# ShuhongChen/panic3d-anime-reconstruction

Hardware: AMD Instinct MI355X
Metric: rendered rays/sec at 512^2 img x 96 samples/ray (higher is better)
Workload: dtype f32

## Files before the change

### panic3d-anime-reconstruction_amd/csrc/p3d_importance.hpp

```cpp
#pragma once

#if defined(__HIPCC__)
#define P3D_IMP_FN __host__ __device__ __forceinline__
#define P3D_IMP_UNROLL _Pragma("unroll")
#else
#define P3D_IMP_FN inline
#define P3D_IMP_UNROLL
#endif

struct P3dFloatKey {
    P3D_IMP_FN static float mn(float a, float b) { return __builtin_fminf(a, b); }
    P3D_IMP_FN static float mx(float a, float b) { return __builtin_fmaxf(a, b); }
    P3D_IMP_FN static float neg(float a) { return -a; }
};

P3D_IMP_FN constexpr int p3d_pow2_ceil(int n) { int p = 1; while (p < n) p <<= 1; return p; }

template <int NR, typename K = P3dFloatKey, typename T>
P3D_IMP_FN void p3d_sort_merge_pass(T (&a)[NR], int pp) {
    constexpr int N = p3d_pow2_ceil(NR);
P3D_IMP_UNROLL
    for (int k = pp; k >= 1; k >>= 1) {
P3D_IMP_UNROLL
        for (int jj = k % pp; jj + k < N; jj += 2 * k) {
P3D_IMP_UNROLL
            for (int i = 0; i < k; ++i) {
                if (i + jj + k < NR && (i + jj) / (2 * pp) == (i + jj + k) / (2 * pp)) {
                    T x = a[i + jj], y = a[i + jj + k];
                    a[i + jj] = K::mn(x, y);
                    a[i + jj + k] = K::mx(x, y);
                }
            }
        }
    }
}
template <int NR, typename K = P3dFloatKey, typename T>
P3D_IMP_FN void p3d_sort_network(T (&a)[NR]) {
P3D_IMP_UNROLL
    for (int pp = 1; pp < p3d_pow2_ceil(NR); pp <<= 1) p3d_sort_merge_pass<NR, K>(a, pp);
}

template <typename K = P3dFloatKey, typename T>
P3D_IMP_FN void p3d_cross_half_exchange(T lo, T hi_neg, T& lo_out_neg, T& hi_out) {
    lo_out_neg = K::mx(K::neg(lo), hi_neg);
    hi_out = K::mx(lo, K::neg(hi_neg));
}

template <int H, typename K = P3dFloatKey, typename T>
P3D_IMP_FN void p3d_valley_merge(T (&a)[H]) {
    constexpr int N = p3d_pow2_ceil(H);
P3D_IMP_UNROLL
    for (int k = N / 2; k >= 1; k >>= 1) {
P3D_IMP_UNROLL
        for (int i = 0; i < H; ++i) {
            if ((i & k) == 0 && i + k < H) {
                T x = a[i], y = a[i + k];
                a[i] = K::mn(x, y);
                a[i + k] = K::mx(x, y);
            }
        }
    }
}

P3D_IMP_FN constexpr int p3d_half_rank(int H, int h, int i) { return h ? H + i : H - 1 - i; }

P3D_IMP_FN int p3d_merge_split_steps(int Sc, int Sf) {
    int n = Sc < Sf ? Sc : Sf, s = 0;
    while (n > 0) { ++s; n >>= 1; }
    return s;
}
template <typename RD>
P3D_IMP_FN int p3d_merge_split(RD rd, int Sc, int Sf, int D, int steps) {
    int lo = D - Sf > 0 ? D - Sf : 0, hi = D < Sc ? D : Sc;
    for (int s = 0; s < steps; ++s) {
        const int mid = (lo + hi) >> 1;
        const int cm = mid < Sc - 1 ? mid : Sc - 1, fm = D - mid - 1 < 0 ? 0 : (D - mid - 1 < Sf ? D - mid - 1 : Sf - 1);
        const bool behind = rd(false, fm) < rd(true, cm);
        const bool open = lo < hi;
        hi = (open && behind) ? mid : hi;
        lo = (open && !behind) ? mid + 1 : lo;
    }
    return lo;
}

template <typename RD, typename KN, typename PUT>
P3D_IMP_FN void p3d_merge_bits_half(RD rd, KN known, PUT put, int Sc, int Sf, int h) {
    const int S = Sc + Sf, D = S >> 1, qb = h ? D : 0, qe = h ? S : D;
    int ci = p3d_merge_split(rd, Sc, Sf, qb, p3d_merge_split_steps(Sc, Sf)), fi = qb - ci;
    const float inf = __builtin_inff();
    float ta = rd(true, ci < Sc ? ci : Sc - 1), tb = Sf > 0 ? rd(false, fi < Sf ? fi : Sf - 1) : inf;
    unsigned kw = 0u, sw = 0u;
    for (int it = 0; it < S - D; ++it) {
        const int q = qb + it;
        const bool mine = q < qe;
        const bool take_c = (ci < Sc) && (fi >= Sf || ta <= tb);
        const bool kn = known(take_c, take_c ? ci : fi, take_c ? ta : tb);
        kw |= (mine && kn) ? (1u << (q & 31)) : 0u;
        sw |= (mine && take_c) ? (1u << (q & 31)) : 0u;
        ci += take_c ? 1 : 0;
        fi += take_c ? 0 : 1;
        const int cq = ci < Sc ? ci : Sc - 1, fq = fi < Sf ? fi : (Sf > 0 ? Sf - 1 : 0);
        const float nv = rd(take_c, take_c ? cq : fq);
        ta = take_c ? nv : ta;
        tb = take_c ? tb : nv;
        if (mine && ((q & 31) == 31 || q == qe - 1)) {
            put(q >> 5, kw, sw);
            kw = 0u; sw = 0u;
        }
    }
}

#if defined(__HIPCC__)
template <int H>
__device__ __forceinline__ void p3d_sort_halves(float (&tf)[H], int h) {
    typedef uint32_t u32x2 __attribute__((ext_vector_type(2)));
    const uint32_t neg1 = h ? 0x80000000u : 0u;
P3D_IMP_UNROLL
    for (int i = 0; i < H; ++i) tf[i] = __builtin_bit_cast(float, __builtin_bit_cast(uint32_t, tf[i]) ^ neg1);
    p3d_sort_network<H>(tf);
P3D_IMP_UNROLL
    for (int i = 0; i < H; i += 2) {
        u32x2 in = __builtin_amdgcn_permlane32_swap(__builtin_bit_cast(uint32_t, tf[i]), __builtin_bit_cast(uint32_t, tf[i + 1]), false, false);
        const uint32_t in0 = in.x, in1 = in.y;
        float mn_neg, mx;
        p3d_cross_half_exchange(__builtin_bit_cast(float, in0), __builtin_bit_cast(float, in1), mn_neg, mx);
        u32x2 out = __builtin_amdgcn_permlane32_swap(__builtin_bit_cast(uint32_t, mn_neg), __builtin_bit_cast(uint32_t, mx), false, false);
        const uint32_t out0 = out.x, out1 = out.y;
        tf[i] = __builtin_bit_cast(float, out0);
        tf[i + 1] = __builtin_bit_cast(float, out1);
    }
    p3d_valley_merge<H>(tf);
}

template <typename RAW>
__device__ __forceinline__ float p3d_coarse_rank(RAW raw, int i, int Sc, bool wave_unsorted, bool wave_bad) {
    float a = raw(i);
    if (wave_unsorted) {
        if (!wave_bad) {
            const float lo = i > 0 ? raw(i - 1) : -__builtin_inff(), hi = i < Sc - 1 ? raw(i + 1) : __builtin_inff();
            a = lo > a ? lo : (a > hi ? hi : a);
        } else {
            for (int c = 0; c < Sc; ++c) {
                const float tv = raw(c);
                int r = 0;
                for (int x = 0; x < Sc; ++x) {
                    const float tx = raw(x);
                    r += (tx < tv || (tx == tv && x < c)) ? 1 : 0;
                }
                a = (r == i) ? tv : a;
            }
        }
    }
    return a;
}

template <typename TCS, typename FINE, typename KN, typename PUT>
__device__ __forceinline__ void p3d_merge_bits_ranks(TCS tc_sorted, FINE fine, KN known, PUT put, uint32_t fw0, uint32_t fw1, uint32_t fw2,
                                                     int Sc, int Sf, int h) {
    const int S = Sc + Sf, nmw = (S + 31) >> 5;
    uint32_t slw[6], knw[6];
P3D_IMP_UNROLL
    for (int w = 0; w < 6; ++w) { slw[w] = 0u; knw[w] = 0u; }
    const int Sch = ((Sc + 15) >> 4) << 3, ib = h * Sch;
    for (int i0 = 0; i0 < Sch; i0 += 8) {
        float tv[8];
        int pos[8];
P3D_IMP_UNROLL
        for (int q = 0; q < 8; ++q) { tv[q] = tc_sorted(ib + i0 + q < Sc ? ib + i0 + q : Sc - 1); pos[q] = 0; }
P3D_IMP_UNROLL
        for (int step = 64; step >= 1; step >>= 1) {
            float c[8];
P3D_IMP_UNROLL
            for (int q = 0; q < 8; ++q) c[q] = fine((pos[q] + step <= Sf) ? pos[q] + step - 1 : 0);
P3D_IMP_UNROLL
            for (int q = 0; q < 8; ++q) pos[q] = ((pos[q] + step <= Sf) && (c[q] < tv[q])) ? pos[q] + step : pos[q];
        }
P3D_IMP_UNROLL
        for (int q = 0; q < 8; ++q) {
            const int i = ib + i0 + q;
            const bool kn = known(i, tv[q]);
            const int P = i + pos[q], pw = (i < Sc) ? (P >> 5) : -1;
            const uint32_t b = 1u << (P & 31);
P3D_IMP_UNROLL
            for (int w = 0; w < 6; ++w) {
                slw[w] |= (pw == w) ? b : 0u;
                knw[w] |= (pw == w && kn) ? b : 0u;
            }
        }
    }
P3D_IMP_UNROLL
    for (int w = 0; w < 6; ++w) { slw[w] |= __shfl_xor(slw[w], 32); knw[w] |= __shfl_xor(knw[w], 32); }
    if (__builtin_amdgcn_ballot_w64((fw0 | fw1 | fw2) != 0u) != 0) {
        int fk = 0;
P3D_IMP_UNROLL
        for (int w = 0; w < 6; ++w) {
            if (w * 32 < S) {
                uint32_t kk = 0u;
                for (int b = 0; b < 32; ++b) {
                    const bool isf = !((slw[w] >> b) & 1u) && (w * 32 + b < S);
                    const uint32_t fwv = (fk < 32) ? fw0 : (fk < 64 ? fw1 : fw2);
                    kk |= (isf && ((fwv >> (fk & 31)) & 1u)) ? (1u << b) : 0u;
                    fk += isf ? 1 : 0;
                }
                knw[w] |= kk;
            }
        }
    }
P3D_IMP_UNROLL
    for (int w = 0; w < 6; ++w)
        if (w < nmw) put(w, knw[w], slw[w]);
}
#endif
```

### panic3d-anime-reconstruction_amd/csrc/p3d_kernels.hip

```cpp
#include <hip/hip_runtime.h>
#include <stddef.h>
#include <stdlib.h>
#include <string.h>

#include <atomic>
#include <type_traits>

#include "p3d_ray_phases.hpp"
#include "p3d_render_plan.hpp"
#include "p3d_phase_timing.hpp"

#define P3D_WAVES_PER_WG 4
#define P3D_WG (64 * P3D_WAVES_PER_WG)

__global__ __launch_bounds__(256) void k_planes_to_nhwc(const float* __restrict__ src, float* __restrict__ dst, int HW) {
    __shared__ float tile[32][65];
    const int p0 = blockIdx.x * 64;
    const size_t img = (size_t)blockIdx.y * 32 * HW;
    {
        int px = threadIdx.x & 63, c0 = threadIdx.x >> 6;
#pragma unroll
        for (int k = 0; k < 8; ++k) {
            int c = c0 + 4 * k;
            tile[c][px] = (p0 + px < HW) ? src[img + (size_t)c * HW + p0 + px] : 0.0f;
        }
    }
    __syncthreads();
    {
        int c = threadIdx.x & 31, q0 = threadIdx.x >> 5;
#pragma unroll
        for (int k = 0; k < 8; ++k) {
            int px = q0 + 8 * k;
            if (p0 + px < HW) dst[img + (size_t)(p0 + px) * 32 + c] = tile[c][px];
        }
    }
}

struct DecodeParams {
    const float* planes;
    const float* coords;
    const float *w0, *b0, *w1, *b1;
    float* out_sigma;
    float* out_rgb;
    unsigned char* out_cropmask;
    float mask_limit;
    long long M;
    long long tiles_per_img;
    long long ntiles;
    int H, W;
    int grid_n;
    long long grid_lo;
    float vsize, goff0, goff1, goff2;
    P3dDecodeCfg cfg;
};

P3D_DEV float p3d_fmod_pos(float a, float b) {
    const float q = __builtin_truncf(a / b);
    const float r = __builtin_fmaf(-q, b, a);
    return r < 0.0f ? r + b : r;
}

template <bool WANT_RGB, bool STAGED, bool FASTD>
__global__ __launch_bounds__(P3D_WG, 2) void k_decode_points(DecodeParams p) {
    static_assert(!(FASTD && WANT_RGB), "the tolerance-mode point decoder is density-only");
    extern __shared__ __attribute__((aligned(16))) float lds_alloc[];
    float* lds = FASTD ? lds_alloc - P3D_LDS_B0P : lds_alloc;
    p3d_load_mlp_to_lds(lds, p.w0, p.b0, p.w1, p.b1, !FASTD, !FASTD);
    if constexpr (FASTD) p3d_load_mlp_f16_to_lds(lds, p.w0, p.w1, false);
    __syncthreads();
    const int lane = threadIdx.x & 63, wave = threadIdx.x >> 6, j = lane & 31, h = lane >> 5;
    float* box = lds + (FASTD ? P3D_LDS_FAST_FLOATS : P3D_LDS_MLP_FLOATS) + 4 + (STAGED ? wave * P3D_BOX_FLOATS_PER_WAVE : 0);
    (void)box;
    P3dPlaneGeom g;
    g.halfW = 0.5f * (float)p.W; g.halfH = 0.5f * (float)p.H; g.fW = (float)p.W; g.fH = (float)p.H; g.W = p.W;
    g.plane_bytes = (uint32_t)p.H * (uint32_t)p.W * 128u;
    const long long stride = (long long)gridDim.x * P3D_WAVES_PER_WG;

    struct Tile {
        long long n, m;
        bool active, skip, any;
        float px, py, pz;
    };
    auto setup = [&](long long tile, Tile& t) {
        long long n = 0, tl = tile;
        if (p.tiles_per_img != p.ntiles) { n = tile / p.tiles_per_img; tl = tile - n * p.tiles_per_img; }
        t.n = n;
        t.m = tl * 32 + j;
        t.active = t.m < p.M;
        const long long mc = t.active ? t.m : p.M - 1;
        t.skip = false;
        if (p.coords) {
            const float* c = p.coords + ((size_t)n * p.M + mc) * 3;
            t.px = c[0]; t.py = c[1]; t.pz = c[2];
        } else {
            const unsigned idx = (unsigned)(p.grid_lo + mc);
            const float fn = (float)p.grid_n, f = (float)idx;
            const float s2 = (float)(idx % (unsigned)p.grid_n);
            const float q1 = f / fn;
            const float s1 = p3d_fmod_pos(q1, fn);
            const float s0 = p3d_fmod_pos(q1 / fn, fn);
            t.px = s0 * p.vsize + p.goff0; t.py = s1 * p.vsize + p.goff1; t.pz = s2 * p.vsize + p.goff2;
            if (p.out_cropmask) {
                const bool cropped = __builtin_fabsf(t.px) > p.mask_limit || __builtin_fabsf(t.pz) > p.mask_limit;
                if (t.active && h == 0) p.out_cropmask[t.m] = cropped ? 1 : 0;
                if (p.cfg.flags & P3D_FLAG_SKIP_CROPPED) t.skip = cropped;
            }
        }
        t.any = __builtin_amdgcn_ballot_w64(t.active && !t.skip) != 0;
    };
    auto resource = [&](long long n) {
        const unsigned nlo = __builtin_amdgcn_readfirstlane((unsigned)n);
        const float* base = p.planes + ((p.cfg.flags & P3D_FLAG_SHARED_PLANES) ? (size_t)0 : (size_t)nlo * 3 * (g.plane_bytes / 4));
        return __builtin_amdgcn_make_buffer_rsrc((void*)base, 0, 3 * g.plane_bytes, 0x00020000);
    };
    auto finish = [&](const Tile& t, float sigma, const f32x16& rgb) {
        if (t.skip) sigma = -1000.0f;
        if (t.active) {
            const size_t o = (size_t)t.n * p.M + t.m;
            if (h == 0) p.out_sigma[o] = sigma;
            if (WANT_RGB) {
                float* dst = p.out_rgb + o * 32 + 4 * h;
#pragma unroll
                for (int q = 0; q < 4; ++q)
                    *(f32x4*)(dst + 8 * q) = (f32x4){rgb[4 * q], rgb[4 * q + 1], rgb[4 * q + 2], rgb[4 * q + 3]};
            }
        }
    };

    long long tile = (long long)blockIdx.x * P3D_WAVES_PER_WG + wave;
    if constexpr (!STAGED) {
        for (; tile < p.ntiles; tile += stride) {
            Tile t;
            setup(tile, t);
            float sigma = -1000.0f;
            f32x16 rgb;
            if (t.any) {
                if constexpr (FASTD) p3d_decode_wave_fast<WANT_RGB, true>(lds, resource(t.n), g, p.cfg, t.px, t.py, t.pz, sigma, rgb, !t.skip);
                else p3d_decode_wave<WANT_RGB>(lds, resource(t.n), g, p.cfg, t.px, t.py, t.pz, sigma, rgb, !t.skip);
            }
            finish(t, sigma, rgb);
        }
    } else {
        if (tile >= p.ntiles) return;
        Tile cur, nxt;
        P3dStage st;
        setup(tile, cur);
        bool cur_staged = cur.any && p3d_stage_plan(resource(cur.n), g, p.cfg, cur.px, cur.py, cur.pz, st);
        for (;;) {
            P3dBox cb[3] = {st.b[0], st.b[1], st.b[2]};
            if (cur_staged) p3d_stage_commit(box, st);
            const long long next = tile + stride;
            bool nxt_staged = false;
            if (next < p.ntiles) {
                setup(next, nxt);
                nxt_staged = nxt.any && p3d_stage_plan(resource(nxt.n), g, p.cfg, nxt.px, nxt.py, nxt.pz, st);
            }
            float sigma = -1000.0f;
            f32x16 rgb;
            if (cur.any) {
                if (cur_staged) {
                    const f32x16 X = p3d_gather_features_boxed(box, cb, g, p.cfg, cur.px, cur.py, cur.pz, !cur.skip);
                    if constexpr (FASTD) p3d_decode_features_fast<WANT_RGB>(lds, p.cfg, X, cur.px, cur.pz, sigma, rgb);
                    else p3d_decode_features<WANT_RGB>(lds, p.cfg, X, cur.px, cur.pz, sigma, rgb);
                } else if constexpr (FASTD) {
                    p3d_decode_wave_fast<WANT_RGB>(lds, resource(cur.n), g, p.cfg, cur.px, cur.py, cur.pz, sigma, rgb, !cur.skip);
                } else {
                    p3d_decode_wave<WANT_RGB>(lds, resource(cur.n), g, p.cfg, cur.px, cur.py, cur.pz, sigma, rgb, !cur.skip);
                }
            }
            finish(cur, sigma, rgb);
            if (next >= p.ntiles) break;
            tile = next;
            cur = nxt;
            cur_staged = nxt_staged;
        }
    }
}

struct DecodeFeatParams {
    const float* feats;
    const float *w0, *b0, *w1, *b1;
    float* out_sigma;
    float* out_rgb;
    long long M, tiles_per_img, ntiles;
    P3dDecodeCfg cfg;
};
__global__ __launch_bounds__(P3D_WG, 2) void k_decode_features(DecodeFeatParams p) {
    extern __shared__ __attribute__((aligned(16))) float lds[];
    p3d_load_mlp_to_lds(lds, p.w0, p.b0, p.w1, p.b1);
    __syncthreads();
    const int lane = threadIdx.x & 63, wave = threadIdx.x >> 6, j = lane & 31, h = lane >> 5;
    const long long stride = (long long)gridDim.x * P3D_WAVES_PER_WG;
    for (long long tile = (long long)blockIdx.x * P3D_WAVES_PER_WG + wave; tile < p.ntiles; tile += stride) {
        const long long n = tile / p.tiles_per_img, m = (tile - n * p.tiles_per_img) * 32 + j;
        const bool active = m < p.M;
        const long long mc = active ? m : p.M - 1;
        f32x16 f[3];
#pragma unroll
        for (int pl = 0; pl < 3; ++pl) {
            const f32x4* src = (const f32x4*)(p.feats + (((size_t)n * 3 + pl) * p.M + mc) * 32 + 16 * h);
#pragma unroll
            for (int q = 0; q < 4; ++q) {
                const f32x4 v = src[q];
                f[pl][4 * q] = v.x; f[pl][4 * q + 1] = v.y; f[pl][4 * q + 2] = v.z; f[pl][4 * q + 3] = v.w;
            }
        }
        f32x16 X, rgb;
#pragma unroll
        for (int c = 0; c < 16; ++c) X[c] = ((f[0][c] + f[1][c]) + f[2][c]) * P3D_THIRD;
        float sigma;
        p3d_decode_features<true>(lds, p.cfg, X, 0.0f, 0.0f, sigma, rgb);
        if (active) {
            const size_t o = (size_t)n * p.M + m;
            if (h == 0) p.out_sigma[o] = sigma;
            float* dst = p.out_rgb + o * 32 + 4 * h;
#pragma unroll
            for (int q = 0; q < 4; ++q) *(f32x4*)(dst + 8 * q) = (f32x4){rgb[4 * q], rgb[4 * q + 1], rgb[4 * q + 2], rgb[4 * q + 3]};
        }
    }
}

#define P3D_NF_EXACT(NF) ((NF) == 48 || (NF) == 96)
template <int NF, bool DUMP, bool FAST, bool EARLY, bool TCG = p3d_render_tcg(NF, DUMP, EARLY)>
__global__ __launch_bounds__(64 * P3D_RENDER_WAVES, p3d_render_occ(NF, TCG)) void k_render(RenderParams p) {
    static_assert(!(DUMP && EARLY), "dumps need every sample decoded");
    static_assert(!TCG || p3d_render_tcg(NF, DUMP, EARLY), "TCG exists only for the production 96-key kernel");
    extern __shared__ __attribute__((aligned(16))) float lds[];
    P3D_PHASE_START();
    p3d_load_mlp_to_lds(lds, p.w0, p.b0, p.w1, p.b1, !FAST);
    if constexpr (FAST) p3d_load_mlp_f16_to_lds(lds, p.w0, p.w1);
    __syncthreads();
    const int lane = threadIdx.x & 63, wave = threadIdx.x >> 6, j = lane & 31, h = lane >> 5;
    const long long tile = p3d_render_wave_tile(p, wave);
    if (tile >= p.ntiles) return;
    P3D_PHASE(P3D_PH_WEIGHTS);
    float* wl = lds + (FAST ? P3D_LDS_FAST_FLOATS : P3D_LDS_MLP_FLOATS) + 4 + (size_t)wave * p.lds_rows * 32;
    const int Sc = p.Sc, Sf = P3D_NF_EXACT(NF) ? NF : p.Sf, S = Sc + Sf;
    const P3dRayCtx cx = p3d_ray_setup(p, p3d_render_tile_ray(p, tile, j), Sc, Sf);
    const bool active = cx.active;
    const size_t ray = cx.ray;
    const float ox = cx.ox, oy = cx.oy, oz = cx.oz, dx = cx.dx, dy = cx.dy, dz = cx.dz;
    constexpr bool early = EARLY;
    int ndec = 0;

    float* tcA = wl;
    float* wcA = TCG ? wl : tcA + Sc * 32;
    float* tfA = (NF > 0) ? wcA : wcA + Sc * 32;
    uint32_t* mkA = (uint32_t*)(wl + (size_t)(p.lds_rows - ((Sc + 31) >> 5)) * 32);
    const int nmw = (S + 31) >> 5;
    uint32_t* knA = TCG ? (uint32_t*)(wl + (size_t)(Sc > Sf ? Sc : Sf) * 32) : mkA - (size_t)2 * nmw * 32;
    uint32_t* slA = knA + (size_t)nmw * 32;
    const P3dSpacing sp = TCG ? p3d_spacing_fixed(p.ray_start, p.ray_end, p.depth_delta, Sc) : p3d_spacing_of(p, ray, Sc);
    auto tc_raw = [&](int i) -> float { return p3d_stratified_fixed(i, Sc, cx.jitter(i), sp); };
    auto tc_of = [&](int i) -> float { if constexpr (TCG) return tc_raw(i); else return tcA[i * 32 + j]; };
    bool wave_unsorted = false;
    bool bad_order = false;
    bool wave_bad = false;
    auto tc_sorted = [&](int i) -> float { return p3d_coarse_rank(tc_raw, i, Sc, wave_unsorted, wave_bad); };
    uint32_t mw0 = 0u, mw1 = 0u, mw2 = 0u;
    uint32_t fw0 = 0u, fw1 = 0u, fw2 = 0u;
    const bool dump = DUMP && active && h == 0;

    bool unsorted = false;
    float tcmin = __builtin_inff(), tcmax = -__builtin_inff();
    if constexpr (!TCG) {
        float prev = -__builtin_inff();
        for (int i0 = 0; i0 < Sc; i0 += 8) {
            float jv[8];
#pragma unroll
            for (int q = 0; q < 8; ++q) jv[q] = cx.jitter(i0 + q < Sc ? i0 + q : Sc - 1);
#pragma unroll
            for (int q = 0; q < 8; ++q) {
                const int i = i0 + q;
                if (i < Sc) {
                    const float t = p3d_stratified_depth(i, Sc, jv[q], sp);
                    tcA[i * 32 + j] = t;
                    unsorted |= (t < prev);
                    prev = t;
                    tcmin = __builtin_fminf(tcmin, t);
                    tcmax = __builtin_fmaxf(tcmax, t);
                    if constexpr (DUMP) if (dump && p.dumps.depths_coarse) p.dumps.depths_coarse[ray * Sc + i] = t;
                }
            }
        }
    }
    P3D_PHASE(P3D_PH_STRAT);
    float tmin = __builtin_inff(), tmax = -__builtin_inff();
    if (Sf > 0) {
        MarchState st = p3d_march_start();
        uint32_t mword = 0;
        if constexpr (TCG) {
            float prev = -__builtin_inff(), pmax = -__builtin_inff();
            for (int i0 = 0; i0 < Sc; i0 += 8) {
                float jv[8];
#pragma unroll
                for (int q = 0; q < 8; ++q) jv[q] = cx.jitter(i0 + q < Sc ? i0 + q : Sc - 1);
#pragma unroll
                for (int q = 0; q < 8; ++q) {
                    const int i = i0 + q;
                    if (i >= Sc) break;
                    const float t = p3d_stratified_fixed(i, Sc, jv[q], sp);
                    unsorted |= (t < prev);
                    bad_order |= (t < pmax);
                    pmax = __builtin_fmaxf(pmax, prev);
                    prev = t;
                    tcmin = __builtin_fminf(tcmin, t);
                    tcmax = __builtin_fmaxf(tcmax, t);
                    const float px = ox + t * dx, py = oy + t * dy, pz = oz + t * dz;
                    float sigma = P3D_SIGMA_MASKED;
                    const bool cropped = cx.cropped(px, pz);
                    const bool live = !(cropped || st.Td < 1e-60);
                    const bool skip = __builtin_amdgcn_ballot_w64(live) == 0;
                    if (!skip) {
                        f32x16 dummy;
                        p3d_decode_wave<false, true>(lds, cx.rs, cx.g, cx.cfg, px, py, pz, sigma, dummy, live);
                    }
                    mword |= (cropped || (live && sigma == P3D_SIGMA_MASKED)) ? (1u << (i & 31)) : 0u;
                    if ((i & 31) == 31 || i == Sc - 1) {
                        if ((i >> 5) == 0) mw0 = mword; else if ((i >> 5) == 1) mw1 = mword; else mw2 = mword;
                        mword = 0;
                    }
                    if (i > 0) wcA[(i - 1) * 32 + j] = p3d_march_interval(st, t, sigma).w;
                    st.prev_t = t; st.prev_sigma = sigma;
                    ndec += skip ? 0 : 1;
                }
            }
        } else
        for (int i = 0; i < Sc; ++i) {
            float t = tcA[i * 32 + j];
            float px = ox + t * dx, py = oy + t * dy, pz = oz + t * dz;
            float sigma = P3D_SIGMA_MASKED;
            bool skip = false, live = true, cropped = false;
            if (early) {
                cropped = cx.cropped(px, pz);
                live = !(cropped || st.Td < 1e-60);
                skip = __builtin_amdgcn_ballot_w64(live) == 0;
            }
            if (!skip) {
                f32x16 dummy;
                p3d_decode_wave<false, true>(lds, cx.rs, cx.g, cx.cfg, px, py, pz, sigma, dummy, live);
            }
            if (early) {
                mword |= (cropped || (live && sigma == P3D_SIGMA_MASKED)) ? (1u << (i & 31)) : 0u;
                if ((i & 31) == 31 || i == Sc - 1) { mkA[(i >> 5) * 32 + j] = mword; mword = 0; }
            }
            if constexpr (DUMP) if (dump && p.dumps.sigma_coarse) p.dumps.sigma_coarse[ray * Sc + i] = sigma;
            if (i > 0) {
                float w = p3d_march_interval(st, t, sigma).w;
                wcA[(i - 1) * 32 + j] = w;
                if constexpr (DUMP) if (dump && p.dumps.weights_coarse) p.dumps.weights_coarse[ray * (Sc - 1) + i - 1] = w;
            }
            st.prev_t = t; st.prev_sigma = sigma;
            if constexpr (!DUMP) ndec += skip ? 0 : 1;
        }
        P3D_PHASE(P3D_PH_COARSE);
        const int Ns = Sc - 3;
        p3d_pdf_to_cdf<32>(wcA, Ns, j);
        P3D_PHASE(P3D_PH_CDF);
        constexpr int DB = P3D_DRAW_BATCH;
        auto dump_draw = [&](bool mine, int i, float v, int k) {
            if constexpr (DUMP) {
                if (mine && p.dumps.depths_fine) p.dumps.depths_fine[ray * Sf + i] = v;
                if (mine && p.dumps.inds) p.dumps.inds[ray * Sf + i] = k;
            }
        };
        if constexpr (P3D_NF_EXACT(NF)) {
            constexpr int H = NF / 2;
            static_assert(H % DB == 0, "whole batches of draws per half");
            const int d0 = h * H;
            float tf[H];
#pragma unroll
            for (int i = 0; i < H; ++i) tf[i] = cx.u(d0 + i);
#pragma unroll
            for (int i0 = 0; i0 < H; i0 += DB) {
                float ub[DB], vb[DB];
                int kb[DB];
#pragma unroll
                for (int q = 0; q < DB; ++q) ub[q] = tf[i0 + q];
                p3d_inverse_cdf<DB, 32>(wcA, tc_of, Ns, j, ub, vb, kb);
#pragma unroll
                for (int q = 0; q < DB; ++q) {
                    tf[i0 + q] = vb[q];
                    dump_draw(active, d0 + i0 + q, vb[q], kb[q]);
                }
            }
            P3D_PHASE(P3D_PH_DRAWS);
            p3d_sort_halves<H>(tf, h);
            __builtin_amdgcn_fence(__ATOMIC_ACQ_REL, "wavefront");
            const int row0 = p3d_half_rank(H, h, 0), rstep = h ? 1 : -1;
            const uint32_t neg0 = h ? 0u : 0x80000000u;
            uint64_t crop = 0ull;
#pragma unroll
            for (int i = 0; i < H; ++i) {
                const float v = __builtin_bit_cast(float, __builtin_bit_cast(uint32_t, tf[i]) ^ neg0);
                tfA[(row0 + rstep * i) * 32 + j] = v;
                if constexpr (TCG) crop |= cx.cropped_at(v) ? (1ull << i) : 0ull;
            }
            __builtin_amdgcn_fence(__ATOMIC_ACQ_REL, "wavefront");
            if constexpr (TCG) {
                static_assert(H >= 32 && H < 64, "the 96 rank bits as 64 + 32");
                const uint64_t g0 = h ? (crop << H) : (__builtin_bitreverse64(crop) >> (64 - H));
                fw0 = (uint32_t)g0; fw1 = (uint32_t)(g0 >> 32); fw2 = h ? (uint32_t)(crop >> (64 - H)) : 0u;
                fw0 |= __shfl_xor(fw0, 32); fw1 |= __shfl_xor(fw1, 32); fw2 |= __shfl_xor(fw2, 32);
            }
        } else if constexpr (NF > 0) {
            float tf[NF];
#pragma unroll
            for (int i = 0; i < NF; ++i) tf[i] = (i < Sf) ? cx.u(i) : 0.0f;
#pragma unroll
            for (int i0 = 0; i0 < NF; i0 += DB) {
                if (i0 < Sf) {
                    float ub[DB], vb[DB];
                    int kb[DB];
#pragma unroll
                    for (int q = 0; q < DB; ++q) ub[q] = tf[i0 + q];
                    p3d_inverse_cdf<DB, 32>(wcA, tc_of, Ns, j, ub, vb, kb);
#pragma unroll
                    for (int q = 0; q < DB; ++q) {
                        tf[i0 + q] = (i0 + q < Sf) ? vb[q] : __builtin_inff();
                        if (i0 + q < Sf) dump_draw(dump, i0 + q, vb[q], kb[q]);
                    }
                } else {
#pragma unroll
                    for (int q = 0; q < DB; ++q) tf[i0 + q] = __builtin_inff();
                }
            }
            P3D_PHASE(P3D_PH_DRAWS);
            p3d_sort_network<NF>(tf);
#pragma unroll
            for (int i = 0; i < NF; ++i)
                if (i < Sf) {
                    tfA[i * 32 + j] = tf[i];
                    if constexpr (TCG) {
                        const uint32_t b = cx.cropped_at(tf[i]) ? (1u << (i & 31)) : 0u;
                        if (i < 32) fw0 |= b; else if (i < 64) fw1 |= b; else fw2 |= b;
                    }
                }
        } else {
            for (int i0 = 0; i0 < Sf; i0 += DB) {
                float ub[DB], vb[DB];
                int kb[DB];
#pragma unroll
                for (int q = 0; q < DB; ++q) ub[q] = cx.u(i0 + q < Sf ? i0 + q : Sf - 1);
                p3d_inverse_cdf<DB, 32>(wcA, tc_of, Ns, j, ub, vb, kb);
#pragma unroll
                for (int q = 0; q < DB; ++q) {
                    if (i0 + q < Sf) {
                        tfA[(i0 + q) * 32 + j] = vb[q];
                        dump_draw(dump, i0 + q, vb[q], kb[q]);
                    }
                }
            }
            P3D_PHASE(P3D_PH_DRAWS);
            p3d_lds_insertion_sort(tfA, Sf, j);
        }
        P3D_PHASE(P3D_PH_SORT);
        if constexpr (TCG) {
            wave_unsorted = __builtin_amdgcn_ballot_w64(unsorted) != 0;
            wave_bad = __builtin_amdgcn_ballot_w64(bad_order) != 0;
            if (wave_unsorted) { mw0 = 0u; mw1 = 0u; mw2 = 0u; }
        } else
        if (__builtin_amdgcn_ballot_w64(unsorted) != 0) {
            p3d_lds_insertion_sort(tcA, Sc, j);
            if (early) {
                for (int i = 0; i < ((Sc + 31) >> 5); ++i) mkA[i * 32 + j] = 0u;
            }
        }
    }
    MarchState st = p3d_march_start();
    P3dAccum acc;
    f32x16 prev_rgb = 0.0f;
    {
        int ci = 0, fi = 0;
        float ta = TCG ? 0.0f : tcA[j], tb = (Sf > 0) ? tfA[j] : __builtin_inff();
        tmin = __builtin_fminf(tcmin, tb);
        tmax = __builtin_fmaxf(tcmax, (Sf > 0) ? tfA[(Sf - 1) * 32 + j] : -__builtin_inff());
        bool prev_skipped = false, first = true, done = false;
        int m = 0;
        auto advance = [&](bool take_c) {
            ci += take_c ? 1 : 0;
            fi += take_c ? 0 : 1;
            const int cq = ci < Sc ? ci : Sc - 1, fq = fi < Sf ? fi : (Sf > 0 ? Sf - 1 : 0);
            const float nv = (take_c ? tcA : tfA)[(take_c ? cq : fq) * 32 + j];
            ta = take_c ? nv : ta;
            tb = take_c ? tb : nv;
        };
        float tcn = 0.0f;
        if constexpr (TCG) {
            p3d_merge_bits_ranks(
                tc_sorted, [&](int k) { return tfA[k * 32 + j]; },
                [&](int i, float t) {
                    const uint32_t mwv = (i < 32) ? mw0 : (i < 64 ? mw1 : mw2);
                    return cx.cropped_at(t) || ((mwv >> (i & 31)) & 1u);
                },
                [&](int w, uint32_t kw, uint32_t sw) { knA[w * 32 + j] = kw; slA[w * 32 + j] = sw; }, fw0, fw1, fw2, Sc, Sf, h);
            tcn = tc_sorted(0);
        } else
        if constexpr (EARLY) {
            for (int w = 0; w < nmw; ++w) { knA[w * 32 + j] = 0u; slA[w * 32 + j] = 0u; }
            __builtin_amdgcn_fence(__ATOMIC_ACQ_REL, "wavefront");
            p3d_merge_bits_half(
                [&](bool c, int i) { return (c ? tcA : tfA)[i * 32 + j]; },
                [&](bool c, int i, float t) {
                    bool known = cx.cropped_at(t);
                    if (c && Sf > 0) known = known || ((mkA[(i >> 5) * 32 + j] >> (i & 31)) & 1u);
                    return known;
                },
                [&](int w, uint32_t kw, uint32_t sw) { atomicOr(&knA[w * 32 + j], kw); atomicOr(&slA[w * 32 + j], sw); },
                Sc, Sf, h);
            __builtin_amdgcn_fence(__ATOMIC_ACQ_REL, "wavefront");
            ci = 0;
        }
        P3D_PHASE(P3D_PH_MERGE);
        for (int it = 0;; ++it) {
            bool take_c, known = false;
            float t;
            if constexpr (!EARLY) {
                if (it >= S) break;
                take_c = (ci < Sc) && (fi >= Sf || ta <= tb);
                t = take_c ? ta : tb;
                advance(take_c);
            } else {
                if (!done && st.Td < (FAST ? 2e-6 : 1e-60)) done = true;
                if (!done && (first || st.prev_sigma <= 602.0f)) {
                    bool any = false, last_c = false;
                    while (m < S) {
                        const int sh = m & 31, left = (32 - sh < S - m) ? 32 - sh : S - m;
                        const uint32_t kw = knA[(m >> 5) * 32 + j] >> sh, sw = slA[(m >> 5) * 32 + j] >> sh;
                        int run = (~kw != 0u) ? __builtin_ctz(~kw) : 32;
                        run = run < left ? run : left;
                        if (run > 0) {
                            const uint32_t inrun = run >= 32 ? 0xffffffffu : ((1u << run) - 1u);
                            ci += __builtin_popcount(sw & inrun);
                            last_c = (sw >> (run - 1)) & 1u;
                            any = true;
                            m += run;
                        }
                        if (run < left) break;
                    }
                    if (any) {
                        if constexpr (TCG) {
                            const float pc = tc_sorted(ci > 0 ? ci - 1 : 0);
                            tcn = tc_sorted(ci < Sc ? ci : Sc - 1);
                            st.prev_t = last_c ? pc : tfA[(m - ci - 1 > 0 ? m - ci - 1 : 0) * 32 + j];
                        } else
                        st.prev_t = last_c ? tcA[(ci - 1) * 32 + j] : tfA[(m - ci - 1) * 32 + j];
                        st.prev_sigma = P3D_SIGMA_MASKED;
                        prev_skipped = true; first = false;
                    }
                    done = m >= S;
                }
                if (__builtin_amdgcn_ballot_w64(!done) == 0) break;
                const int mm = done ? S - 1 : m;
                const uint32_t kb = knA[(mm >> 5) * 32 + j] >> (mm & 31), sb = slA[(mm >> 5) * 32 + j] >> (mm & 31);
                take_c = (sb & 1u) != 0u;
                known = !done && (kb & 1u) != 0u;
                const int cq = ci < Sc ? ci : Sc - 1, fq = (m - ci < Sf) ? m - ci : (Sf > 0 ? Sf - 1 : 0);
                if constexpr (TCG) t = take_c ? tcn : tfA[fq * 32 + j];
                else t = (take_c || Sf == 0) ? tcA[cq * 32 + j] : tfA[fq * 32 + j];
                if (!done) { ++m; ci += take_c ? 1 : 0; }
                if constexpr (TCG) {
                    if (!done && take_c) tcn = tc_sorted(ci < Sc ? ci : Sc - 1);
                }
            }
            P3D_PHASE(P3D_PH_SELECT);
            const bool have = EARLY ? !done : true;
            const float px = ox + t * dx, py = oy + t * dy, pz = oz + t * dz;
            float sigma = P3D_SIGMA_MASKED;
            f32x16 rgb = 0.0f;
            const bool live = have && !known;
            bool skipped = true;
            if (__builtin_amdgcn_ballot_w64(live) != 0) {
                bool have_rgb;
                if constexpr (FAST) have_rgb = p3d_decode_wave_fast<true, true, EARLY, true>(lds, cx.rs, cx.g, cx.cfg, px, py, pz, sigma, rgb, live);
                else have_rgb = p3d_decode_wave<true, true, EARLY>(lds, cx.rs, cx.g, cx.cfg, px, py, pz, sigma, rgb, live);
                if constexpr (!DUMP) ndec += 1;
                skipped = !live || !have_rgb;
                if (known) sigma = P3D_SIGMA_MASKED;
            }
            P3D_PHASE(P3D_PH_DECODE);
            if constexpr (DUMP) {
                if (dump && p.dumps.depths_sorted) p.dumps.depths_sorted[ray * S + m] = t;
                if (dump && p.dumps.sigma_sorted) p.dumps.sigma_sorted[ray * S + m] = sigma;
            }
            const bool marching = have && !first;
            P3dInterval iv = {0.0f, 0.0f, 0.0f, 0.0f};
            if (marching) iv = p3d_march_interval(st, t, sigma);
            const float ppx = ox + st.prev_t * dx, ppy = oy + st.prev_t * dy, ppz = oz + st.prev_t * dz;
            if (early) p3d_guard_colours<FAST>(lds, cx, marching, iv.w, prev_skipped, prev_rgb, ppx, ppy, ppz, skipped, rgb, px, py, pz);
            if (have) {
                if (!first) p3d_composite_interval<false>(acc, st, iv, prev_rgb, rgb, ppx, ppy, ppz, px, py, pz);
                st.prev_t = t; st.prev_sigma = sigma;
                prev_rgb = rgb;
                prev_skipped = skipped;
                first = false;
                if constexpr (!EARLY) ++m;
            }
            P3D_PHASE(P3D_PH_MARCH);
        }
    }
    p3d_ray_outputs<false, DUMP>(p, ray, h, active, acc, st);
    p3d_wave_minmax(active, tmin, tmax);
    P3D_PHASE(P3D_PH_OUT);
    P3D_PHASE_FLUSH();
    p3d_depth_range_atomics<!DUMP>(p, cx.nlo, lane, tmin, tmax, ndec);
}

template <int X>
P3D_DEV float p3d_lane_xor(float v) {
    return __builtin_bit_cast(float, __builtin_amdgcn_ds_swizzle(__builtin_bit_cast(int, v), 0x1f | (X << 10)));
}

template <int N>
P3D_DEV float p3d_select(const float (&x)[N], int k) {
    static_assert(N == 2 || N == 4, "two or four entries");
    const float x0 = x[0], x1 = x[1];
    if constexpr (N == 2) {
        return (k & 1) ? x1 : x0;
    } else {
        const float x2 = x[2], x3 = x[3];
        return (k & 2) ? ((k & 1) ? x3 : x2) : ((k & 1) ? x1 : x0);
    }
}

template <int SLOTS, int NF, bool FAST, bool WO = false>
__global__ __launch_bounds__(64 * P3D_RENDER_WAVES, p3d_render_slots_occ(SLOTS, FAST)) void k_render_slots(RenderParams p) {
    static_assert(SLOTS == 2 || SLOTS == 4, "16 rays x 2 slots or 8 rays x 4 slots per wave");
    static_assert(!WO || (FAST && SLOTS == 4), "the weights-only launch exists for the tolerance mode (the renderer class's default, what the paste runs)");
    constexpr int RPW = 32 / SLOTS;
    constexpr int RS = RPW;
    extern __shared__ __attribute__((aligned(16))) float lds[];
    p3d_load_mlp_to_lds(lds, p.w0, p.b0, p.w1, p.b1, !FAST);
    if constexpr (FAST) p3d_load_mlp_f16_to_lds(lds, p.w0, p.w1);
    __syncthreads();
    const int lane = threadIdx.x & 63, wave = threadIdx.x >> 6, j = lane & 31, h = lane >> 5;
    const int jr = j % RPW, slot = j / RPW;
    const int nwaves = blockDim.x >> 6;
    long long tile = (long long)blockIdx.x * nwaves + wave;
    if (tile >= p.ntiles) return;
    float* wl = lds + (FAST ? P3D_LDS_FAST_FLOATS : P3D_LDS_MLP_FLOATS) + 4 + (size_t)wave * p.lds_rows * RS;
    const int Sc = p.Sc, Sf = P3D_NF_EXACT(NF) ? NF : p.Sf, S = Sc + Sf;
    const P3dRayCtx cx = p3d_ray_setup(p, p3d_slots_tile_ray<RPW>(p, tile, jr), Sc, Sf);
    const bool active = cx.active;
    const size_t ray = cx.ray;
    const float ox = cx.ox, oy = cx.oy, oz = cx.oz, dx = cx.dx, dy = cx.dy, dz = cx.dz;
    const bool early = !(cx.cfg.flags & P3D_FLAG_NO_EARLY_OUT);
    int ndec = 0;
    struct Slots { float x0, x1, x2, x3; };
    auto exchange = [](float v) {
        Slots s{v, p3d_lane_xor<RPW>(v), v, v};
        if constexpr (SLOTS == 4) { s.x2 = p3d_lane_xor<2 * RPW>(v); s.x3 = p3d_lane_xor<3 * RPW>(v); }
        return s;
    };
    auto of_slot = [&](int q, Slots s) {
        const int k = slot ^ q;
        return (k & 1) ? ((k & 2) ? s.x3 : s.x1) : ((k & 2) ? s.x2 : s.x0);
    };

    float* tcA = wl;
    float* wcA = tcA + Sc * RS;
    float* tfA = (NF > 0) ? wcA : wcA + Sc * RS;
    auto tc_lds = [&](int i) { return tcA[i * RS + jr]; };

    bool unsorted = false;
    {
        const P3dSpacing sp = p3d_spacing_of(p, ray, Sc);
        float prev = -__builtin_inff();
        for (int i = 0; i < Sc; ++i) {
            const float t = p3d_stratified_depth(i, Sc, cx.jitter(i), sp);
            tcA[i * RS + jr] = t;
            unsorted |= (t < prev);
            prev = t;
        }
    }
    float tmin = __builtin_inff(), tmax = -__builtin_inff();
    if (Sf > 0) {
        MarchState st = p3d_march_start();
        for (int i = 0; i < Sc; i += SLOTS) {
            float tq[SLOTS];
#pragma unroll
            for (int q = 0; q < SLOTS; ++q) tq[q] = tcA[(i + q < Sc ? i + q : Sc - 1) * RS + jr];
            const float t = p3d_select(tq, slot);
            const float px = ox + t * dx, py = oy + t * dy, pz = oz + t * dz;
            float sigma = P3D_SIGMA_MASKED;
            bool skip = false, live = true;
            if (early) {
                live = !(cx.cropped(px, pz) || st.Td < 1e-60);
                skip = __builtin_amdgcn_ballot_w64(live) == 0;
            }
            if (!skip) {
                f32x16 dummy;
                p3d_decode_wave<false, true>(lds, cx.rs, cx.g, cx.cfg, px, py, pz, sigma, dummy, live);
                ndec += 1;
            }
            const Slots sx = exchange(sigma);
#pragma unroll
            for (int q = 0; q < SLOTS; ++q) {
                if (i + q < Sc) {
                    const float sq = of_slot(q, sx);
                    if (i + q > 0) wcA[(i + q - 1) * RS + jr] = p3d_march_interval(st, tq[q], sq).w;
                    st.prev_t = tq[q]; st.prev_sigma = sq;
                }
            }
        }
        const int Ns = Sc - 3;
        p3d_pdf_to_cdf<RS>(wcA, Ns, jr);
        if constexpr (NF > 0) {
            float tf[NF];
            constexpr int DB = P3D_DRAW_BATCH;
#pragma unroll
            for (int i = 0; i < NF; ++i) tf[i] = (i < Sf) ? cx.u(i) : 0.0f;
#pragma unroll
            for (int i0 = 0; i0 < NF; i0 += DB) {
                if (i0 < Sf) {
                    float ub[DB], vb[DB];
                    int kb[DB];
#pragma unroll
                    for (int q = 0; q < DB; ++q) ub[q] = tf[i0 + q];
                    p3d_inverse_cdf<DB, RS>(wcA, tc_lds, Ns, jr, ub, vb, kb);
#pragma unroll
                    for (int q = 0; q < DB; ++q) tf[i0 + q] = (i0 + q < Sf) ? vb[q] : __builtin_inff();
                } else {
#pragma unroll
                    for (int q = 0; q < DB; ++q) tf[i0 + q] = __builtin_inff();
                }
            }
            p3d_sort_network<NF>(tf);
#pragma unroll
            for (int i = 0; i < NF; ++i)
                if (i < Sf) tfA[i * RS + jr] = tf[i];
        } else {
            for (int i = 0; i < Sf; ++i) {
                const float ui[1] = {cx.u(i)};
                float v[1];
                int k[1];
                p3d_inverse_cdf<1, RS>(wcA, tc_lds, Ns, jr, ui, v, k);
                tfA[i * RS + jr] = v[0];
            }
            if (slot == 0 && h == 0) p3d_lds_insertion_sort<RS>(tfA, Sf, jr);
        }
        if (__builtin_amdgcn_ballot_w64(unsorted) != 0 && slot == 0 && h == 0) p3d_lds_insertion_sort<RS>(tcA, Sc, jr);
    }
    MarchState st = p3d_march_start();
    P3dAccum acc;
    f32x16 prev_rgb = 0.0f;
    float ppx = 0.0f, ppy = 0.0f, ppz = 0.0f;
    {
        int ci = 0, fi = 0;
        float ta = tcA[jr], tb = (Sf > 0) ? tfA[jr] : __builtin_inff();
        bool prev_skipped = false;
        auto next_depth = [&]() {
            const bool take_c = (ci < Sc) && (fi >= Sf || ta <= tb);
            const float t = take_c ? ta : tb;
            ci += take_c ? 1 : 0;
            fi += take_c ? 0 : 1;
            const int cq = ci < Sc ? ci : Sc - 1, fq = fi < Sf ? fi : (Sf > 0 ? Sf - 1 : 0);
            const float nv = (take_c ? tcA : tfA)[(take_c ? cq : fq) * RS + jr];
            ta = take_c ? nv : ta;
            tb = take_c ? tb : nv;
            tmin = __builtin_fminf(tmin, t);
            tmax = __builtin_fmaxf(tmax, t);
            return t;
        };
        auto consume = [&](int m, float t, float px, float py, float pz, float sigma, f32x16 rgb, bool skipped) {
            if (m > 0) {
                const P3dInterval iv = p3d_march_interval(st, t, sigma);
                if (early && !WO) p3d_guard_colours<FAST>(lds, cx, true, iv.w, prev_skipped, prev_rgb, ppx, ppy, ppz, skipped, rgb, px, py, pz);
                p3d_composite_interval<WO>(acc, st, iv, prev_rgb, rgb, ppx, ppy, ppz, px, py, pz);
            }
            st.prev_t = t; st.prev_sigma = sigma;
            prev_rgb = rgb;
            prev_skipped = skipped;
            ppx = px; ppy = py; ppz = pz;
        };
        for (int m = 0; m < S; m += SLOTS) {
            float tq[SLOTS], pxq[SLOTS], pyq[SLOTS], pzq[SLOTS];
#pragma unroll
            for (int q = 0; q < SLOTS; ++q) {
                tq[q] = (m + q < S) ? next_depth() : tq[q > 0 ? q - 1 : 0];
                pxq[q] = ox + tq[q] * dx; pyq[q] = oy + tq[q] * dy; pzq[q] = oz + tq[q] * dz;
            }
            const float px = p3d_select(pxq, slot), py = p3d_select(pyq, slot), pz = p3d_select(pzq, slot);
            float sigma = P3D_SIGMA_MASKED;
            f32x16 rgb = 0.0f;
            bool skipped = false, live = true;
            if (early) {
                live = !(cx.cropped(px, pz) || st.Td < (FAST ? 2e-6 : 1e-60));
                skipped = __builtin_amdgcn_ballot_w64(live) == 0;
            }
            if (!skipped) {
                if constexpr (FAST) p3d_decode_wave_fast<!WO, true, false, true>(lds, cx.rs, cx.g, cx.cfg, px, py, pz, sigma, rgb, live);
                else p3d_decode_wave<true, true>(lds, cx.rs, cx.g, cx.cfg, px, py, pz, sigma, rgb, live);
                ndec += 1;
                skipped = !live;
            }
            const Slots sx = exchange(sigma), kx = exchange(skipped ? 1.0f : 0.0f);
            f32x16 r1 = rgb, r2 = rgb, r3 = rgb;
            if constexpr (!WO) {
#pragma unroll
                for (int c = 0; c < 16; ++c) { const Slots x = exchange(rgb[c]); r1[c] = x.x1; r2[c] = x.x2; r3[c] = x.x3; }
            }
            consume(m, tq[0], pxq[0], pyq[0], pzq[0], of_slot(0, sx), rgb, of_slot(0, kx) != 0.0f);
            if (m + 1 < S) consume(m + 1, tq[1], pxq[1], pyq[1], pzq[1], of_slot(1, sx), r1, of_slot(1, kx) != 0.0f);
            if constexpr (SLOTS == 4) {
                if (m + 2 < S) consume(m + 2, tq[2], pxq[2], pyq[2], pzq[2], of_slot(2, sx), r2, of_slot(2, kx) != 0.0f);
                if (m + 3 < S) consume(m + 3, tq[3], pxq[3], pyq[3], pzq[3], of_slot(3, sx), r3, of_slot(3, kx) != 0.0f);
            }
        }
    }
    p3d_ray_outputs<WO, false>(p, ray, h, active && slot == 0, acc, st);
    p3d_wave_minmax(active, tmin, tmax);
    p3d_depth_range_atomics<true>(p, cx.nlo, lane, tmin, tmax, ndec);
}

__global__ void k_minmax_init(uint32_t* g, int nviews) {
    const int i = blockIdx.x * blockDim.x + threadIdx.x;
    if (i == 0) {
        g[0] = 0xffffffffu;
        g[1] = 0u;
        g[2] = 0u;
        g[3] = 0u;
    }
    if (i < nviews) { g[4 + 2 * i] = 0xffffffffu; g[5 + 2 * i] = 0u; }
}

__global__ void k_render_finish(float* depth, long long n, const uint32_t* g, float* dump_tminmax, long long rays_per_view) {
    long long i = (long long)blockIdx.x * blockDim.x + threadIdx.x;
    if (i == 0 && dump_tminmax) { dump_tminmax[0] = p3d_ord2f(g[0]); dump_tminmax[1] = p3d_ord2f(g[1]); }
    if (i < n) {
        const uint32_t* mm = rays_per_view > 0 ? g + 4 + 2 * (i / rays_per_view) : g;
        const float lo = p3d_ord2f(mm[0]), hi = p3d_ord2f(mm[1]);
        float d = depth[i];
        d = d < lo ? lo : d;
        d = d > hi ? hi : d;
        depth[i] = d;
    }
}

__global__ void k_stratified(float start, float end, float delta, int S, const float* __restrict__ jitter, long long NR,
                             float* __restrict__ out) {
    long long r = (long long)blockIdx.x * blockDim.x + threadIdx.x;
    if (r >= NR) return;
    const P3dSpacing sp = p3d_spacing_fixed(start, end, delta, S);
    for (int i = 0; i < S; ++i) out[r * S + i] = p3d_stratified_fixed(i, S, jitter[r * S + i], sp);
}

__global__ void k_minmax_decode(const uint32_t* g, float* out) {
    out[0] = p3d_ord2f(g[0]);
    out[1] = p3d_ord2f(g[1]);
}

__global__ void k_depth_minmax(const float* __restrict__ d, long long n, uint32_t* g) {
    float lo = __builtin_inff(), hi = -__builtin_inff();
    for (long long i = (long long)blockIdx.x * blockDim.x + threadIdx.x; i < n; i += (long long)gridDim.x * blockDim.x) {
        lo = __builtin_fminf(lo, d[i]);
        hi = __builtin_fmaxf(hi, d[i]);
    }
    p3d_wave_minmax(true, lo, hi);
    if ((threadIdx.x & 63) == 0) {
        atomicMin(g, p3d_f2ord(lo));
        atomicMax(g + 1, p3d_f2ord(hi));
    }
}

__global__ void k_composite(const float* __restrict__ colors, const float* __restrict__ sigma,
                            const float* __restrict__ depths, long long NR, int S, int K, int white_back,
// ... 486 lines not shown
```

Baseline: 86.63 million.

## Split stratified depth generation across half-waves and cache merge bitmask words in registers

```diff
diff --git a/panic3d-anime-reconstruction_amd/csrc/p3d_importance.hpp b/panic3d-anime-reconstruction_amd/csrc/p3d_importance.hpp
--- a/panic3d-anime-reconstruction_amd/csrc/p3d_importance.hpp
+++ b/panic3d-anime-reconstruction_amd/csrc/p3d_importance.hpp
@@ -110,6 +110,30 @@
     }
 }
 
+P3D_IMP_FN constexpr int p3d_stratified_cut(int Sc) { return Sc >> 1; }
+template <int B = 8, typename DEPTH, typename PUT>
+P3D_IMP_FN void p3d_stratified_half(DEPTH depth, PUT put, int Sc, int cut, int h, bool& unsorted, float& tmin, float& tmax) {
+    const int b = h ? cut : 0, e = h ? Sc : cut, n = cut > Sc - cut ? cut : Sc - cut;
+    const float front = depth(cut > 0 ? cut - 1 : 0);
+    float prev = (h && cut > 0) ? front : -__builtin_inff();
+    for (int i0 = 0; i0 < n; i0 += B) {
+        float t[B];
+P3D_IMP_UNROLL
+        for (int q = 0; q < B; ++q) t[q] = depth(b + i0 + q < Sc ? b + i0 + q : Sc - 1);
+P3D_IMP_UNROLL
+        for (int q = 0; q < B; ++q) {
+            const int i = b + i0 + q;
+            if (i < e) {
+                put(i, t[q]);
+                unsorted |= (t[q] < prev);
+                prev = t[q];
+                tmin = __builtin_fminf(tmin, t[q]);
+                tmax = __builtin_fmaxf(tmax, t[q]);
+            }
+        }
+    }
+}
+
 #if defined(__HIPCC__)
 template <int H>
 __device__ __forceinline__ void p3d_sort_halves(float (&tf)[H], int h) {
diff --git a/panic3d-anime-reconstruction_amd/csrc/p3d_kernels.hip b/panic3d-anime-reconstruction_amd/csrc/p3d_kernels.hip
--- a/panic3d-anime-reconstruction_amd/csrc/p3d_kernels.hip
+++ b/panic3d-anime-reconstruction_amd/csrc/p3d_kernels.hip
@@ -264,25 +264,14 @@
     bool unsorted = false;
     float tcmin = __builtin_inff(), tcmax = -__builtin_inff();
     if constexpr (!TCG) {
-        float prev = -__builtin_inff();
-        for (int i0 = 0; i0 < Sc; i0 += 8) {
-            float jv[8];
-#pragma unroll
-            for (int q = 0; q < 8; ++q) jv[q] = cx.jitter(i0 + q < Sc ? i0 + q : Sc - 1);
-#pragma unroll
-            for (int q = 0; q < 8; ++q) {
-                const int i = i0 + q;
-                if (i < Sc) {
-                    const float t = p3d_stratified_depth(i, Sc, jv[q], sp);
-                    tcA[i * 32 + j] = t;
-                    unsorted |= (t < prev);
-                    prev = t;
-                    tcmin = __builtin_fminf(tcmin, t);
-                    tcmax = __builtin_fmaxf(tcmax, t);
-                    if constexpr (DUMP) if (dump && p.dumps.depths_coarse) p.dumps.depths_coarse[ray * Sc + i] = t;
-                }
-            }
-        }
+        p3d_stratified_half<8>(
+            [&](int i) { return p3d_stratified_depth(i, Sc, cx.jitter(i), sp); },
+            [&](int i, float t) {
+                tcA[i * 32 + j] = t;
+                if constexpr (DUMP) if (active && p.dumps.depths_coarse) p.dumps.depths_coarse[ray * Sc + i] = t;
+            },
+            Sc, p3d_stratified_cut(Sc), h, unsorted, tcmin, tcmax);
+        __builtin_amdgcn_fence(__ATOMIC_ACQ_REL, "wavefront");
     }
     P3D_PHASE(P3D_PH_STRAT);
     float tmin = __builtin_inff(), tmax = -__builtin_inff();
@@ -497,7 +486,8 @@
             tcn = tc_sorted(0);
         } else
         if constexpr (EARLY) {
-            for (int w = 0; w < nmw; ++w) { knA[w * 32 + j] = 0u; slA[w * 32 + j] = 0u; }
+            typedef uint32_t u32x4 __attribute__((ext_vector_type(4)));
+            for (int x = lane * 4; x < 2 * nmw * 32; x += 256) *(u32x4*)(knA + x) = (u32x4){0u, 0u, 0u, 0u};
             __builtin_amdgcn_fence(__ATOMIC_ACQ_REL, "wavefront");
             p3d_merge_bits_half(
                 [&](bool c, int i) { return (c ? tcA : tfA)[i * 32 + j]; },
@@ -511,6 +501,15 @@
             __builtin_amdgcn_fence(__ATOMIC_ACQ_REL, "wavefront");
             ci = 0;
         }
+        uint32_t kwr = 0u, swr = 0u;
+        float tcp = 0.0f, tfp = 0.0f;
+        auto load_words = [&]() { kwr = knA[(m >> 5) * 32 + j]; swr = slA[(m >> 5) * 32 + j]; };
+        auto load_heads = [&]() {
+            const int cq = ci < Sc ? ci : Sc - 1, fq = (m - ci < Sf) ? m - ci : (Sf > 0 ? Sf - 1 : 0);
+            if constexpr (!TCG) tcp = tcA[cq * 32 + j];
+            tfp = (Sf > 0 ? tfA : wl)[fq * 32 + j];
+        };
+        if constexpr (EARLY) { load_words(); load_heads(); }
         P3D_PHASE(P3D_PH_MERGE);
         for (int it = 0;; ++it) {
             bool take_c, known = false;
@@ -521,12 +520,12 @@
                 t = take_c ? ta : tb;
                 advance(take_c);
             } else {
-                if (!done && st.Td < (FAST ? 2e-6 : 1e-60)) done = true;
+                if (!done && (m >= S || st.Td < (FAST ? 2e-6 : 1e-60))) done = true;
                 if (!done && (first || st.prev_sigma <= 602.0f)) {
                     bool any = false, last_c = false;
                     while (m < S) {
                         const int sh = m & 31, left = (32 - sh < S - m) ? 32 - sh : S - m;
-                        const uint32_t kw = knA[(m >> 5) * 32 + j] >> sh, sw = slA[(m >> 5) * 32 + j] >> sh;
+                        const uint32_t kw = kwr >> sh, sw = swr >> sh;
                         int run = (~kw != 0u) ? __builtin_ctz(~kw) : 32;
                         run = run < left ? run : left;
                         if (run > 0) {
@@ -537,6 +536,7 @@
                             m += run;
                         }
                         if (run < left) break;
+                        if (m < S) load_words();
                     }
                     if (any) {
                         if constexpr (TCG) {
@@ -545,23 +545,25 @@
                             st.prev_t = last_c ? pc : tfA[(m - ci - 1 > 0 ? m - ci - 1 : 0) * 32 + j];
                         } else
                         st.prev_t = last_c ? tcA[(ci - 1) * 32 + j] : tfA[(m - ci - 1) * 32 + j];
+                        load_heads();
                         st.prev_sigma = P3D_SIGMA_MASKED;
                         prev_skipped = true; first = false;
                     }
                     done = m >= S;
                 }
                 if (__builtin_amdgcn_ballot_w64(!done) == 0) break;
-                const int mm = done ? S - 1 : m;
-                const uint32_t kb = knA[(mm >> 5) * 32 + j] >> (mm & 31), sb = slA[(mm >> 5) * 32 + j] >> (mm & 31);
-                take_c = (sb & 1u) != 0u;
-                known = !done && (kb & 1u) != 0u;
-                const int cq = ci < Sc ? ci : Sc - 1, fq = (m - ci < Sf) ? m - ci : (Sf > 0 ? Sf - 1 : 0);
-                if constexpr (TCG) t = take_c ? tcn : tfA[fq * 32 + j];
-                else t = (take_c || Sf == 0) ? tcA[cq * 32 + j] : tfA[fq * 32 + j];
-                if (!done) { ++m; ci += take_c ? 1 : 0; }
+                take_c = ((swr >> (m & 31)) & 1u) != 0u;
+                known = !done && ((kwr >> (m & 31)) & 1u) != 0u;
+                if constexpr (TCG) t = take_c ? tcn : tfp;
+                else t = (take_c || Sf == 0) ? tcp : tfp;
+                if (!done) {
+                    ++m; ci += take_c ? 1 : 0;
+                    if ((m & 31) == 0 && m < S) load_words();
+                }
                 if constexpr (TCG) {
                     if (!done && take_c) tcn = tc_sorted(ci < Sc ? ci : Sc - 1);
                 }
+                load_heads();
             }
             P3D_PHASE(P3D_PH_SELECT);
             const bool have = EARLY ? !done : true;
```

New measurement: 87.15 million (median of 6 runs). No clear change (+0.6%).
